# Matrixeigs/PowerSystemsReliabilityAssessment

Hardware: AMD Instinct MI355X
Metric: Monte Carlo DC-OPF scenarios/sec (RTS-24 HL2 non-sequential) (higher is better)
Workload: dtype f64

## Files before the change

### powersystemsreliabilityassessment_amd/_lib.py

```python
from __future__ import annotations

import ctypes as C
import os
import subprocess

from . import _abi

_CSRC = os.path.join(os.path.dirname(os.path.abspath(__file__)), "csrc")
LIB_PATH = os.environ.get("RELMC_LIB_PATH") or os.path.join(_CSRC, "librelmc.so")

EXPORTS = [
    "relmc_ctx_create", "relmc_ctx_destroy", "relmc_last_error", "relmc_version",
    "relmc_solver_opts_default", "relmc_nsq_opts_default", "relmc_case_load",
    "relmc_case_thresholds", "relmc_mc_sampling", "relmc_mc_sampling_dev",
    "relmc_mc_simulation", "relmc_mc_simulation_dev", "relmc_nsq_accumulate", "relmc_nsq_accumulate_distinct",
    "relmc_last_kernel_ms", "relmc_acc_zero", "relmc_acc_merge", "relmc_nsq_indices",
    "relmc_nsq_run", "relmc_hl1_load", "relmc_hl1_nsq", "relmc_hl1_seq_load", "relmc_hl1_seq", "relmc_hl1_seq_events",
    "relmc_hl1_plan_load", "relmc_hl1_plan", "relmc_hl1_area_load", "relmc_hl1_area", "relmc_hl1_area_tie_outages",
    "relmc_comm_unique_id", "relmc_comm_init", "relmc_comm_allreduce_acc", "relmc_comm_destroy", "relmc_comm_set_host_allreduce", "relmc_comm_info",
    "relmc_db_reset", "relmc_nsq_db_batch", "relmc_db_accumulate", "relmc_db_size", "relmc_db_export", "relmc_db_import",
    "relmc_seq_load", "relmc_seq_mcsampling", "relmc_seq_mcsimulation", "relmc_seq_years", "relmc_retry_stats", "relmc_retry_overflow", "relmc_retry_dense_stats", "relmc_case_order",
    "relmc_case_order_hint", "relmc_tune_order",
    "relmc_comm_set_timeout", "relmc_comm_allreduce_f64", "relmc_comm_set_host_allreduce_f64", "relmc_device_pci_bus_id", "relmc_seq_opts_default", "relmc_seq_run",
]
# ... 159 lines not shown
    L.relmc_tune_order.argtypes = [C.c_void_p, C.c_int32, C.c_uint64, i32p, i32p, i32p]
    L.relmc_tune_order.restype = C.c_int32
    L.relmc_db_export.argtypes = [vp, C.c_int64, C.c_int64, u8p, _abi.c_int64_p, dp, i32p, dp, i32p, i32p, u8p]
    L.relmc_db_export.restype = C.c_int32
    L.relmc_db_import.argtypes = [vp, C.c_void_p, C.c_int64, u8p, _abi.c_int64_p, dp, dp, i32p, i32p, u8p]
    L.relmc_db_import.restype = C.c_int32
    if hasattr(L, "relmc_debug_screen_states"):
        L.relmc_debug_screen_states.argtypes = [vp, u8p, dp, C.c_int64, u8p]
        L.relmc_debug_screen_states.restype = C.c_int32
    if hasattr(L, "relmc_debug_stretch_len"):
        L.relmc_debug_stretch_len.argtypes = [C.c_int64, C.c_int64, C.c_double, C.c_double, C.c_int64, i32p]
        L.relmc_debug_stretch_len.restype = C.c_int64
    if hasattr(L, "relmc_debug_set"):
        L.relmc_debug_set.argtypes = [vp, C.c_char_p, C.c_int32]
        L.relmc_debug_set.restype = C.c_int32
    if hasattr(L, "relmc_dpp_probe"):
        L.relmc_dpp_probe.argtypes = [vp, dp, dp]
        L.relmc_dpp_probe.restype = C.c_int32
    _lib = L
    return L
```

### powersystemsreliabilityassessment_amd/api.py

```python
from __future__ import annotations

import ctypes as C
from dataclasses import dataclass, field

import numpy as np

from . import _abi, _lib, case24

REFERENCE_EMULATE = _abi.RELMC_REFERENCE_EMULATE
PHYSICAL = _abi.RELMC_PHYSICAL


class RelmcError(RuntimeError):
    pass


def mpoption(singular_policy: int = REFERENCE_EMULATE, **overrides) -> _abi.SolverOpts:
    o = _abi.default_solver_opts(singular_policy)
    for k, v in overrides.items():
        if not hasattr(o, k):
            raise TypeError(f"unknown solver option {k!r}")
        setattr(o, k, v)
    return o

# ... 313 lines not shown
    def pci_bus_id(self) -> str:
        buf = C.create_string_buffer(64)
        self._check(self.L.relmc_device_pci_bus_id(self._h, buf, 64), "relmc_device_pci_bus_id")
        return buf.value.decode()

    def debug_set(self, key: str, value: bool = True):
        self._check(self.L.relmc_debug_set(self._h, key.encode(), int(bool(value))), "relmc_debug_set")

    def shape_path(self) -> str:
        f = self.L.relmc_debug_shape_path
        f.restype, f.argtypes = C.c_int32, [C.c_void_p]
        rc = f(self._h)
        if rc < 0:
            raise RelmcError(f"relmc_debug_shape_path failed ({rc})")
        return "static" if rc == 1 else "dynamic"

    def last_kernel_ms(self) -> float:
        ms = C.c_double()
        self._check(self.L.relmc_last_kernel_ms(self._h, C.byref(ms)), "relmc_last_kernel_ms")
        return ms.value

    def indices(self, acc: _abi.Acc, hours_per_year: float = 8760.0) -> _abi.Indices:
        out = _abi.Indices()
        self.L.relmc_nsq_indices(C.byref(acc), self.case.nb, self.case.ncomp, hours_per_year, C.byref(out))
        return out

    def nsqMain(self, beta_limit: float = 0.0017, max_iterations: int = 100000,
                samples_per_batch: int = 100, *, seed: int = 1, mpopt=None,
                hours_per_year: float = 8760.0, distinct_states: bool | int | str = False, verbose: bool = False) -> NsqResult:
        o = _abi.NsqOpts()
# ... 52 lines not shown
```

### powersystemsreliabilityassessment_amd/csrc/relmc_core.hip

```cpp
#include <hip/hip_runtime.h>

#include <cmath>
#include <cstddef>
#include <cstdio>
#include <cstdlib>
#include <cstring>
#include <memory>
#include <new>
#include <type_traits>

#include "relmc_ctx.h"
#ifdef RELMC_DEV_SWITCHES
#include "relmc_dev_switches.h"
#endif
#include "relmc_kernels.hip"

static_assert(sizeof(relmc::DevAcc) == sizeof(relmc_acc), "device accumulator image must match relmc_acc");

namespace relmc_host {

const char* const kNoCtx = "relmc: null context";

int fail(relmc_ctx* ctx, int code, const std::string& msg)
{
// ... 33 lines not shown
        HIP_TRY(ctx, ctx->retry.dense.grow(need));
        a.dense = ctx->retry.dense.get(); a.dense_stride = stride;
    }
    HIP_TRY(ctx, ctx->dpartial.grow(sizeof(PartialT<TL>) * 64 * TL::WPB * (size_t)blocks));
    a.partial = ctx->dpartial.get();
    a.scen_doubles = alt ? ctx->alt_scen_doubles[alt - 1] : ctx->scen_doubles;
    a.prio_mode = blocks != ctx->num_cu * ctx->blocks_per_cu ? 0u : (ctx->blocks_per_cu == 2 ? 1u : (ctx->blocks_per_cu == 1 && TL::WPB >= 8 ? 2u : 0u));
    a.stash_off = alt ? ctx->alt_stash_off[alt - 1] : ctx->stash_off;
    a.case_bytes = (uint32_t)offsetof(DevCaseT<TL>, task);
#if defined(RELMC_PHASE_TIMING) || defined(RELMC_TRACE)
    HIP_TRY(ctx, ctx->dtiming.grow(8 * 65536));
    a.timing = ctx->dtiming.get(); ctx->timing_waves = blocks * TL::WPB;
#else
    a.timing = nullptr;
#endif
    HIP_TRY(ctx, hipEventRecord(ev_start ? ev_start : ctx->ev0, ctx->stream));
    bool launched = false;
    if constexpr (MODE == 0 && std::is_same<TL, Tile24>::value) {
        if (alt == 0 && ctx->shape_static && !ctx->sw.dynamic_shape) {
            hipLaunchKernelGGL((relmc_eval_kernel<0, Tile24, ShapeRts24>), dim3(blocks), dim3(64 * Tile24::WPB), ctx->lds_bytes, ctx->stream,
                               reinterpret_cast<const DevCaseT<Tile24>*>(ctx->dcase.get()), a);
            launched = true;
        }
    }
    if (!launched)
        hipLaunchKernelGGL((relmc_eval_kernel<MODE, TL>), dim3(blocks), dim3(64 * TL::WPB), alt ? ctx->alt_lds_bytes[alt - 1] : ctx->lds_bytes, ctx->stream,
                           reinterpret_cast<const DevCaseT<TL>*>(alt ? ctx->dcase_alt[alt - 1].get() : ctx->dcase.get()), a);
    HIP_TRY(ctx, hipGetLastError());
    HIP_TRY(ctx, hipEventRecord(ev_stop ? ev_stop : ctx->ev1, ctx->stream));
    *rows_out = blocks * TL::WPB * TL::SPW;
    return RELMC_OK;
}

template <class TL>
int launch_eval_mode(relmc_ctx* ctx, int mode, EvalArgs& a, int* rows_out, hipEvent_t e0, hipEvent_t e1, int alt)
{
    switch (mode) {
        case 0: return launch_eval_t<0, TL>(ctx, a, rows_out, e0, e1, alt);
        case 1: return launch_eval_t<1, TL>(ctx, a, rows_out, e0, e1, alt);
        case 2: return launch_eval_t<2, TL>(ctx, a, rows_out, e0, e1, alt);
        case 3: return launch_eval_t<3, TL>(ctx, a, rows_out, e0, e1, alt);
        case 4: return launch_eval_t<4, TL>(ctx, a, rows_out, e0, e1, alt);
        case 5: return launch_eval_t<5, TL>(ctx, a, rows_out, e0, e1, alt);
// ... 102 lines not shown
    return case_load_impl<Tile96>(ctx, d, *C, order_variant);
}

namespace {
constexpr int64_t kProbeSamples = 8192;
int order_probe(relmc_ctx* ctx, int alt, int32_t* failures)
{
    relmc_solver_opts o; relmc_solver_opts_default(&o);
    EvalArgs a = make_args(o);
    a.seed = 0x5eedca5eull; a.first_index = 0; a.n = kProbeSamples;
    {
        const int rc0 = fail_list_ensure(ctx, fail_cap_for(kProbeSamples));
        if (rc0) return rc0;
    }
    auto& R = ctx->retry;
    HIP_TRY(ctx, hipMemsetAsync(R.fail_count.get(), 0, sizeof(uint32_t), ctx->stream));
    a.fail_list = R.fail.get(); a.fail_count = R.fail_count.get(); a.fail_cap = (uint32_t)R.fail.size(); a.unit_base = 0;
    int rows = 0;
    int rc = launch_eval(ctx, 5, a, &rows, nullptr, nullptr, alt);
    if (rc) return rc;
    uint32_t cnt = 0;
    HIP_TRY(ctx, hipMemcpyAsync(&cnt, R.fail_count.get(), sizeof(cnt), hipMemcpyDeviceToHost, ctx->stream));
    HIP_TRY(ctx, hipStreamSynchronize(ctx->stream));
    HIP_TRY(ctx, hipMemset(R.fail_count.get(), 0, sizeof(uint32_t)));
    R.fail_dirty = false;
    *failures = (int32_t)cnt;
    return RELMC_OK;
}

int order_calibrate(relmc_ctx* ctx)
{
    ctx->order_primary = 0; ctx->order_probe[0] = ctx->order_probe[1] = ctx->order_probe[2] = -1;
    if (ctx->sw.no_retry) return RELMC_OK;
    int rc = order_probe(ctx, 0, &ctx->order_probe[0]);
    if (rc) return rc;
    if ((int64_t)ctx->order_probe[0] * 1000 <= kProbeSamples) return RELMC_OK;
    int best = 0;
    for (int v = 0; v < relmc_ctx::kAlt; ++v) {
        if (alt_ensure(ctx, v) != RELMC_OK) continue;
// ... 257 lines not shown
```

### powersystemsreliabilityassessment_amd/csrc/relmc_ctx.h

```cpp
#pragma once
#include <hip/hip_runtime.h>

#include <cmath>
#include <cstdint>
#include <functional>
#include <string>
#include <vector>

#include "../../include/relmc.h"
#include "relmc_dev.h"

struct relmc_switches {
    bool no_retry = false;
    bool retry_dense_first = false;
    bool nsq_no_stretch = false;
    bool db_no_probe = false;
    bool dynamic_shape = false;
};

namespace relmc_host {
template <class T, bool Pinned = false>
class Buffer {
public:
    Buffer() = default;
    Buffer(Buffer&& o) noexcept : p_(o.p_), n_(o.n_) { o.p_ = nullptr; o.n_ = 0; }
    Buffer& operator=(Buffer&& o) noexcept
    {
        if (this != &o) { reset(); p_ = o.p_; n_ = o.n_; o.p_ = nullptr; o.n_ = 0; }
        return *this;
    }
    ~Buffer() { reset(); }
    T* get() const { return p_; }
// ... 29 lines not shown
    relmc_switches sw;
    struct SeqStep {
        DevBuf<uint32_t> dm, counts, off;
        DevBuf<uint16_t> hours; DevBuf<double> curt, year;
    } sq;
    std::vector<int32_t> order_hint;
    hipStream_t stream = nullptr;
    hipEvent_t ev0 = nullptr, ev1 = nullptr;
    bool has_case = false;
    int tile = 0;
    relmc::DevCaseT<relmc::Tile24> hcase24;
    relmc::DevCaseT<relmc::Tile96> hcase96;
    DevBuf<uint8_t> dcase;
    int nb = 0, ng = 0, nl = 0, ncomp = 0;
    DevBuf<uint8_t> dpartial;
    DevBuf<relmc::DevAcc> dacc;
    struct HostStage { relmc_acc acc; uint32_t fail_cnt, pad; };
    PinBuf<HostStage> hstage;
    int num_cu = 0;
    int blocks_per_cu = 0;
    uint32_t scen_doubles = 0, lds_bytes = 0, stash_off = 0;
    bool shape_static = false;
    DevBuf<unsigned long long> dtiming; int timing_waves = 0;
    struct History { DevBuf<double> d; PinBuf<double> h; } hist;
    struct Memo {
        DevBuf<uint32_t> k, perm0, perm1, head, uid, start, nu;
        DevBuf<unsigned long long> ch0, ch1; DevBuf<uint8_t> tmp;
        DevBuf<uint32_t> miss, k2;
    } memo;
    struct Database {
// ... 1 lines not shown
        DevBuf<uint32_t> keys; DevBuf<unsigned long long> count; DevBuf<double> dns; DevBuf<int32_t> meta; DevBuf<double> nodal; DevBuf<uint32_t> table;
        DevBuf<relmc::DevAcc> partial;
        DevBuf<unsigned long long> snap;
        bool has_opts = false; relmc_solver_opts opts = {};
        bool invalid = false;
    } db;
    struct CaseCopy {
        relmc_case_desc d; bool valid = false;
        std::vector<double> bus_pd, inj_pmin, inj_pmax, inj_cost, br_b, br_rate, unavail; std::vector<int32_t> inj_bus, br_from, br_to; std::vector<uint8_t> always_up;
    } case_copy;
    static constexpr int kAlt = 2;
    int alt_state[kAlt] = {0, 0};
    DevBuf<uint8_t> dcase_alt[kAlt]; uint32_t alt_scen_doubles[kAlt] = {0, 0}, alt_lds_bytes[kAlt] = {0, 0}, alt_stash_off[kAlt] = {0, 0};
    struct Retry {
        DevBuf<relmc::FailRec> fail; DevBuf<uint32_t> fail_count; bool fail_dirty = false;
        DevBuf<double> dense;
        DevBuf<uint32_t> keys; DevBuf<double> dns; DevBuf<int32_t> meta; DevBuf<double> nodal, scale; int64_t rows = 0;
    } retry;
    int64_t retry_dense_units = 0, retry_dense_converged = 0;
    int64_t retry_overflow = 0;
    std::vector<double> hlf;
    int64_t retry_units = 0, retry_converged = 0;
    int order_primary = 0; int32_t order_probe[3] = {-1, -1, -1};
    struct HostPipe {
        bool ready = false; int ncomp = 0, nb = 0;
        hipStream_t up = nullptr, down = nullptr;
        hipEvent_t e_up[2] = {nullptr, nullptr}, e_ks[2] = {nullptr, nullptr}, e_ke[2] = {nullptr, nullptr}, e_down[2] = {nullptr, nullptr};
        struct Bufs {
            DevBuf<uint8_t> d_st; DevBuf<double> d_sc, d_dns, d_nod; DevBuf<int32_t> d_stat, d_it;
            PinBuf<uint8_t> h_st; PinBuf<double> h_sc, h_dns, h_nod; PinBuf<int32_t> h_stat, h_it;
// ... 79 lines not shown
int case_symbolic(const relmc_case_desc* d, DevCaseT<TL>& C, int order_variant, const SymOpts& so, SymGeom& geom, std::string& err);
extern template int case_symbolic<Tile24>(const relmc_case_desc*, DevCaseT<Tile24>&, int, const SymOpts&, SymGeom&, std::string&);
extern template int case_symbolic<Tile96>(const relmc_case_desc*, DevCaseT<Tile96>&, int, const SymOpts&, SymGeom&, std::string&);
inline bool fits_tile24(const relmc_case_desc* d)
{
    return d->nb <= Tile24::NBT && d->nl <= Tile24::NLT && d->ng + d->nd <= Tile24::NIT && d->ng + d->nl <= Tile24::NCOMPMAX;
}

EvalArgs make_args(const relmc_solver_opts& o);
int launch_eval(relmc_ctx* ctx, int mode, EvalArgs& a, int* rows_out, hipEvent_t ev_start = nullptr, hipEvent_t ev_stop = nullptr, int alt = 0);
int launch_finalize(relmc_ctx* ctx, int rows);
int finish_timing(relmc_ctx* ctx);
int case_load_image(relmc_ctx* ctx, const relmc_case_desc* d, int order_variant);
inline int mask_words(const relmc_ctx* ctx) { return ctx->tile == 0 ? Tile24::OW : Tile96::OW; }

constexpr uint32_t kFailCapMin = 4096, kFailCapSteady = 1u << 20, kFailCapMax = 1u << 26;
uint32_t fail_cap_for(int64_t call_units);
int fail_list_ensure(relmc_ctx* ctx, uint32_t cap);
struct RetryOut { std::vector<FailRec> rec; std::vector<double> dns, nodal; std::vector<int32_t> meta; };
int alt_ensure(relmc_ctx* ctx, int v);
int fail_arm(relmc_ctx* ctx, EvalArgs& a, int64_t unit_base, bool reset, int64_t call_units);
int fail_listed(relmc_ctx* ctx, uint32_t* cnt);
using ScaleFn = std::function<double(unsigned long long)>;
int fail_retry(relmc_ctx* ctx, const relmc_solver_opts& o, double fail_threshold, const ScaleFn* scale, RetryOut& out, double* ms, const uint32_t* known_count = nullptr);
void acc_add_unit(relmc_acc* acc, const FailRec& rec, double dns, int32_t meta, const double* nodal, int nb, int ncomp, double fail_threshold);

int pipe_run(relmc_ctx* ctx, const uint8_t* states, const double* load_scale, int64_t n, const relmc_solver_opts& o, double fail_threshold,
             double* dns, double* nodal, int32_t* status, int32_t* iters);
int nsq_accumulate_impl(relmc_ctx* ctx, uint64_t seed, uint64_t first_index, int64_t n, const relmc_solver_opts* opts, relmc_acc* acc_out, double* dns_dev);

constexpr int64_t kStretch = 1 << 18, kStretchMaxBatch = 32768;
inline int64_t stretch_per(int64_t batch) { return kStretch / batch * batch; }
struct Stretch { int64_t len; bool final; };
// ... 38 lines not shown
```

### powersystemsreliabilityassessment_amd/csrc/relmc_debug.hip

```cpp
#include <cstdio>
#include <cstring>
#include <memory>

#include "relmc_ctx.h"
#include "relmc_shape_rts24.h"

using namespace relmc_host;

extern "C" {

int32_t relmc_debug_schedule(const relmc_ctx* ctx, int32_t* out9)
{
    if (!ctx || !out9 || !ctx->has_case) return RELMC_ERR_INVALID;
    auto fill = [&](const auto& C) {
        int ntask = 0;
        for (int p = 0; p < C.npass; ++p) ntask += C.pass_ntask[p];
        out9[0] = C.npass_upd; out9[1] = C.npass_inv; out9[2] = C.npass - C.npass_upd - C.npass_inv; out9[3] = C.noff;
        out9[4] = C.nzero; out9[5] = (int)C.nws; out9[6] = (int)ctx->lds_bytes; out9[7] = ctx->blocks_per_cu; out9[8] = ntask;
        if (verbose()) fprintf(stderr, "relmc: modelled LDS conflict cycles per Newton step %ld -> %ld\n", ctx->conflict_before, ctx->conflict_after);
        if (verbose()) fprintf(stderr, "relmc: longest line / injection list per bus slot: %d %d / %d %d\n", (int)C.maxdeg_s[0], (int)C.maxdeg_s[1], (int)C.maxinj_s[0], (int)C.maxinj_s[1]);
        if (verbose()) { fprintf(stderr, "relmc: tasks per pass:"); for (int p = 0; p < C.npass; ++p) fprintf(stderr, " %d", (int)C.pass_ntask[p]); fprintf(stderr, "\n"); }
    };
    if (ctx->tile == 0) fill(ctx->hcase24); else fill(ctx->hcase96);
    return RELMC_OK;
// ... 76 lines not shown

int64_t relmc_debug_stretch_len(int64_t batch, int64_t done, double beta, double beta_limit, int64_t round, int32_t* final_out)
{
    if (batch <= 0 || batch > kStretchMaxBatch || done < 0 || round < 0) return RELMC_ERR_INVALID;
    const Stretch s = stretch_length(batch, done, beta, beta_limit, stretch_per(batch), round);
    if (final_out) *final_out = s.final ? 1 : 0;
    return s.len;
}

int32_t relmc_debug_shape_path(const relmc_ctx* ctx)
{
    if (!ctx || !ctx->has_case) return RELMC_ERR_INVALID;
    return ctx->shape_static && !ctx->sw.dynamic_shape ? 1 : 0;
}

int32_t relmc_debug_set(relmc_ctx* ctx, const char* key, int32_t value)
{
    if (!ctx || !key) return RELMC_ERR_INVALID;
    const bool v = value != 0;
    if (!std::strcmp(key, "no_retry")) ctx->sw.no_retry = v;
    else if (!std::strcmp(key, "retry_dense_first")) ctx->sw.retry_dense_first = v;
    else if (!std::strcmp(key, "nsq_no_stretch")) ctx->sw.nsq_no_stretch = v;
    else if (!std::strcmp(key, "db_no_probe")) ctx->sw.db_no_probe = v;
    else if (!std::strcmp(key, "dynamic_shape")) ctx->sw.dynamic_shape = v;
    else return fail(ctx, RELMC_ERR_INVALID, std::string("relmc_debug_set: unknown switch ") + key);
    return RELMC_OK;
}

}
```

### powersystemsreliabilityassessment_amd/csrc/relmc_dev.h

```cpp
#pragma once
#include <stdint.h>

namespace relmc {

template <int RW_, int BS_, int LS_, int IS_, int NCOMPMAX_, int MAXPASS_, int MAXOFF_, int WPB_>
struct TileT {
    static constexpr int RW = RW_;
    static constexpr int BS = BS_;
    static constexpr int LS = LS_;
    static constexpr int IS = IS_;
    static constexpr int NBT = BS_ * RW_;
    static constexpr int NLT = LS_ * RW_;
    static constexpr int NIT = IS_ * RW_;
    static constexpr int SPW = 64 / RW_;
    static constexpr int NCOMPMAX = NCOMPMAX_;
    static constexpr int OW = NCOMPMAX_ / 32;
    static constexpr int MAXPASS = MAXPASS_;
    static constexpr int MAXOFF = MAXOFF_;
    static constexpr int WPB = WPB_;
    static_assert(BS_ <= 2 && LS_ <= 3 && IS_ <= 4, "the per-lane flag word has room for 2 bus, 3 line and 4 injection slots");
};
using Tile24 = TileT<16, 2, 3, 4, 128, 96, 160, 4>;
using Tile96 = TileT<64, 2, 2, 3, 256, 64, 320, 8>;
constexpr int DEGMAX = 8;
// ... 37 lines not shown
    uint16_t zero_off[MAXOFF];
    uint8_t pass_ntask[MAXPASS];
    uint16_t task[MAXPASS][ROWL][4];
};

template <class TL>
struct PartialT {
    double dns, dns2;
    double shed[TL::IS];
    uint32_t n, nfail, nsing, ninf, nnc, iters;
    uint32_t cf_inj[TL::IS];
    uint32_t cf_line[TL::LS];
    uint32_t pad;
};

struct FailRec {
    unsigned long long unit;
    uint32_t weight, pad;
    uint32_t mask[8];
};

struct EvalArgs {
    uint64_t seed, first_index;
    int64_t n;
    int32_t policy, max_it;
    double feastol, gradtol, comptol, costtol, xi, sigma, z0, alpha_min, max_stepsize;
    const uint8_t* states;
    double* dns;
    double* nodal;
    int32_t* status;
// ... 7 lines not shown
    double fail_threshold;
    const double* load_scale;
    const uint32_t* seq_masks;
    const uint32_t* seq_offsets;
    const uint16_t* seq_hours;
    const double* load_factors;
    double* curt;
    int32_t seq_nyears, seq_hpy;
    const uint32_t* memo_keys;
    const uint32_t* memo_perm;
    const uint32_t* memo_start;
    int64_t db_first;
    uint32_t* fail_count;
    FailRec* fail_list;
    uint32_t fail_cap;
    int64_t unit_base;
    double* dense;
    uint64_t dense_stride;
};

struct ScreenTab {
    int32_t nl, ng, valid, pad;
    double total_load;
    double sum_pmin, sum_rng;
    const double* pmin;
    const double* rng;
    const double* f_min;
    const double* f_rng;
    const double* f_load;
    const double* lim;
    const double* gpair;
    const double* hmat;
    const uint8_t* bridge;
// ... 75 lines not shown
```

### powersystemsreliabilityassessment_amd/csrc/relmc_kernels.hip

```cpp
#include "relmc_devfn.h"
#include "relmc_shape_rts24.h"

namespace relmc {


constexpr int kPrioBit = 12;
constexpr int kMinWaves = 2;
#define DINF __builtin_inf()
#define RELOAD_FENCE() __asm__ volatile("" ::: "memory")
#define SLOT_FENCE() __builtin_amdgcn_sched_barrier(0)
#ifdef RELMC_PASS_NOUNROLL
#define PASS_LOOP _Pragma("nounroll")
#else
#define PASS_LOOP
#endif
constexpr int kPfMask = 0xc0;
constexpr int kPfMaskWide = 0xc6;
#define PFSITE(k) (((PF_MASK >> (k)) & 1) != 0)
#ifdef RELMC_PHASE_TIMING
#define PT_DECL unsigned long long pt_[8] = {0, 0, 0, 0, 0, 0, 0, 0}; unsigned long long pt0_ = __builtin_readcyclecounter();
#define PT_MARK(k) { const unsigned long long n_ = __builtin_readcyclecounter(); pt_[k] += n_ - pt0_; pt0_ = n_; }
#define PT_FLUSH if (a.timing && lane == 0) { for (int k = 0; k < 8; ++k) a.timing[((size_t)blockIdx.x * WPB + (tid >> 6)) * 8 + k] = pt_[k]; }
#else
#define PT_DECL
// ... 91 lines not shown
    PT_DECL
    const int64_t ngroups = (a.n + SPW - 1) / SPW;
    const int64_t gwave = (int64_t)blockIdx.x * WPB + (tid >> 6);
    const int64_t gstride = (int64_t)gridDim.x * WPB;
    const bool prio_first = a.prio_mode == 1 ? blockIdx.x < (gridDim.x >> 1) : (a.prio_mode == 2 ? ((tid >> 8) & 1) == 0 : false);
    if (a.prio_mode != 0 && !prio_first) __builtin_amdgcn_s_setprio(1);
    constexpr bool WINDOWED = (MODE == 0 && RW == 16);
    uint32_t* const WIN = reinterpret_cast<uint32_t*>(smem + OPT_BYTES + ((case_bytes + 15u) & ~15u)) +
                          (size_t)SPW * WPB * SHAPE(scen_doubles, a.scen_doubles) * 2 + (size_t)(tid >> 6) * 256;
    uint8_t* const WINL = reinterpret_cast<uint8_t*>(smem + OPT_BYTES + ((case_bytes + 15u) & ~15u)) +
                          ((size_t)SPW * WPB * SHAPE(scen_doubles, a.scen_doubles) * 2 + (size_t)WPB * 256) * 4 + (size_t)(tid >> 6) * 64;
    int64_t wb_begin = gwave, wb_end = ngroups, wb_step = gstride;
    if (WINDOWED) {
        wb_begin = ngroups * gwave / gstride; wb_end = ngroups * (gwave + 1) / gstride; wb_step = 16;
    }
    for (int64_t wb = wb_begin; wb < wb_end; wb += wb_step) {
    int win_groups = 1;
    uint32_t win_valid = 0;
    if (WINDOWED) {
        const int64_t si = wb * 4 + lane;
        const bool valid = (wb + (lane >> 2)) < wb_end && si < a.n;
        uint32_t m0 = 0, m1 = 0, m2 = 0, m3 = 0;
        bool hard = false;
        if (valid) {
            const uint64_t gi = a.first_index + (uint64_t)si;
            const int nblk = (ncomp + 3) >> 2;
            for (int blk = 0; blk < nblk; ++blk) {
                uint32_t w[4], nib = 0;
                philox4x32_10((uint32_t)gi, (uint32_t)(gi >> 32), (uint32_t)blk, 0u, (uint32_t)a.seed, (uint32_t)(a.seed >> 32), w);
#pragma unroll
                for (int e = 0; e < 4; ++e) {
                    const int k = blk * 4 + e;
                    if (k < ncomp && w[e] < C.thr[k]) nib |= 1u << e;
                }
// ... 8 lines not shown
            }
            hard = cap * base < C.total_load;
        }
        const uint64_t bv = __ballot(valid), bh = __ballot(valid && hard);
        const uint64_t below = (1ull << lane) - 1ull;
        const uint32_t n_valid = (uint32_t)__popcll(bv), n_easy = (uint32_t)__popcll(bv & ~bh);
        if (valid) {
            const uint32_t slot = hard ? n_easy + (uint32_t)__popcll(bh & below) : (uint32_t)__popcll(bv & ~bh & below);
            uint4 pk; pk.x = m0; pk.y = m1; pk.z = m2; pk.w = m3;
            *reinterpret_cast<uint4*>(WIN + 4 * slot) = pk;
            WINL[slot] = (uint8_t)lane;
        }
        RELOAD_FENCE();
        win_valid = n_valid;
        win_groups = (int)((n_valid + 3u) >> 2);
    }
    PT_IMARK(0)
    for (int wg = 0; wg < win_groups; ++wg) {
        const int64_t grp = WINDOWED ? wb + wg : wb;
        const int64_t sidx = grp * SPW + lane / RW;
        const bool live = WINDOWED ? (uint32_t)(wg * 4 + lane / RW) < win_valid : sidx < a.n;
        double lscale = 1.0;
        uint32_t wgt = 1;
        int seq_year = 0, seq_hour = 0;
        RELOAD_FENCE();

        uint32_t sf = 0;
#define L_ON(s) (((sf >> (s)) & 1u) != 0)
#define L_ACT(s) (((sf >> (3 + (s))) & 1u) != 0)
#define I_ON(s) (((sf >> (6 + (s))) & 1u) != 0)
#define I_BOX(s) (((sf >> (10 + (s))) & 1u) != 0)
#define B_PIN(t) (((sf >> (14 + (t))) & 1u) != 0)
#define B_DROP(t) (((sf >> (16 + (t))) & 1u) != 0)
// ... 883 lines not shown
                    }
#pragma unroll
                    for (int t = 0; t < BS; ++t) {
                        bth[t] = __builtin_fma(alphap, dth[t], bth[t]); bla[t] = __builtin_fma(alphad, dla[t], bla[t]);
                        if (vb[t] < nb) Lam[vb[t]] = bla[t];
                    }
                    zmu = row_sum<RW>(zl);
                    fval = row_sum<RW>(fl);
                    if (niq > 0) gamma = (PFSITE(6) ? o_sg : A_(5, sigma)) * zmu / (double)niq;
                }
                PT_MARK(6)
            }
        }

        PT_MARK(6)
        if (live) {
            double dns = fval + C.total_load * lscale;
            if (dns < 0.1) dns = 0.0;
            const bool fail = dns > a.fail_threshold;
            bool defer = false;
            if (a.fail_list && (status == 1 || status == 2)) {
                uint32_t pos = 0;
                if (rlane == 0) pos = atomicAdd(a.fail_count, 1u);
                pos = __shfl(pos, lane & ~(RW - 1));
                if (pos < a.fail_cap) {
                    defer = true;
                    FailRec* fr = a.fail_list + pos;
                    if (rlane < OW) fr->mask[rlane] = OB[rlane];
                    if (rlane == 0) {
                        const int64_t u = (MODE == 0 && WINDOWED) ? wb * 4 + WINL[wg * 4 + lane / RW]
// ... 1 lines not shown
                                          : (MODE == 7 ? (int64_t)a.memo_perm[sidx]
                                          : (MODE == 4 && a.memo_perm ? (int64_t)a.memo_perm[sidx] : sidx)));
                        fr->unit = (unsigned long long)(u + a.unit_base); fr->weight = wgt; fr->pad = 0;
                    }
                }
            }
            double shed[IS];
#pragma unroll
            for (int s = 0; s < IS; ++s) {
                const int j = RW * s + rlane;
                shed[s] = 0.0;
                if (((iinfo[s] >> 8) & 0xff) == IK_VIRTUAL && dns > 0.0) {
                    const double v = ip[s] * base - C.i_tab[j][3] * lscale;
                    if (v > 1e-3) shed[s] = v;
                }
                if (MODE != 4 && !defer && shed[s] != 0.0) PA.shed[s] += MODE == 3 ? shed[s] * (double)wgt : shed[s];
                if (MODE != 4 && !defer && fail && ((iinfo[s] >> 8) & 0xff) == IK_REAL && outbit(OB, j)) PA.cf_inj[s] += wgt;
            }
#pragma unroll
            for (int s = 0; s < LS; ++s)
                if (MODE != 4 && !defer && fail && ((linfo[s] >> 24) & LF_EXISTS) && outbit(OB, ng + RW * s + rlane)) PA.cf_line[s] += wgt;
            if (MODE != 4 && !defer && rlane == 0) {
                acc_n += wgt;
                if (dns != 0.0) {
                    if (MODE == 3) { PA.dns = __builtin_fma((double)wgt, dns, PA.dns); PA.dns2 = __builtin_fma((double)wgt * dns, dns, PA.dns2); }
                    else { PA.dns += dns; PA.dns2 = __builtin_fma(dns, dns, PA.dns2); }
                }
                if (fail) PA.nfail += wgt;
                if (status == 3) PA.nsing += wgt;
                if (status == 1 || status == 2) PA.nnc += wgt;
                if (infeas) PA.ninf += wgt;
                acc_it += (uint32_t)it * wgt;
            }
            if (MODE == 2 && rlane == 0) a.curt[(size_t)seq_year * a.seq_hpy + seq_hour] = dns;
            if (MODE == 0 && a.dns && rlane == 0)
                a.dns[WINDOWED ? wb * 4 + WINL[wg * 4 + lane / RW] : sidx] = dns;
            if (MODE == 7 && a.dns && rlane == 0) a.dns[a.memo_perm[sidx]] = dns;
            if (MODE == 1 || MODE == 4) {
                const int64_t oidx = MODE == 4 ? a.db_first + (a.memo_perm ? (int64_t)a.memo_perm[sidx] : sidx) : sidx;
#pragma unroll
                for (int s = 0; s < IS; ++s) if (RW * s + rlane < nip) IR[4 * (RW * s + rlane)] = shed[s];
                if (rlane == 0) {
                    a.dns[oidx] = dns;
                    if (MODE == 4) a.status[oidx] = status | (infeas ? 4 : 0) | (it << 8);
                    else {
                        if (a.status) a.status[oidx] = status;
                        if (a.iters) a.iters[oidx] = it;
                    }
                }
                if (a.nodal) {
#pragma unroll
                    for (int t = 0; t < BS; ++t) {
                        const int i = vb[t];
                        if (i < nb) {
                            const int vj = C.b_vinj[i];
                            a.nodal[oidx * nb + C.b_ext[i]] = vj >= 0 ? IR[4 * vj] : 0.0;
                        }
                    }
                }
            }
        }
        PT_MARK(7)
    }
    }
    if (rlane == 0) { PA.n = acc_n; PA.iters = acc_it; }
    PT_FLUSH
}

constexpr int FIN_THREADS = 256, FIN_UNROLL = 8;
template <class TL>
__global__ void __launch_bounds__(FIN_THREADS) relmc_finalize_kernel(const DevCaseT<TL>* __restrict__ C, const PartialT<TL>* __restrict__ part,
                                                                     int nrows, DevAcc* __restrict__ out)
{
    constexpr int RW = TL::RW;
    using Partial = PartialT<TL>;
    const int item = blockIdx.x, tid = threadIdx.x;
    int ln = 0; size_t foff = 0;
    bool is_int = true, active = true;
    if (item < 6) foff = offsetof(Partial, n) + sizeof(uint32_t) * (size_t)item;
    else if (item < 8) { foff = item == 6 ? offsetof(Partial, dns) : offsetof(Partial, dns2); is_int = false; }
    else if (item < 8 + 256) {
// ... 92 lines not shown
```

### powersystemsreliabilityassessment_amd/csrc/relmc_retry.hip

```cpp
#include <algorithm>
#include <cstring>

#include "relmc_ctx.h"

namespace relmc_host {

uint32_t fail_cap_for(int64_t call_units)
{
    const int64_t c = (int64_t)kFailCapMin + call_units / 256;
    return c > (int64_t)kFailCapSteady ? kFailCapSteady : (uint32_t)c;
}
int fail_list_ensure(relmc_ctx* ctx, uint32_t cap)
{
    auto& R = ctx->retry;
    if (!R.fail_count.get()) {
        HIP_TRY(ctx, R.fail_count.grow(1));
        HIP_TRY(ctx, hipMemsetAsync(R.fail_count.get(), 0, sizeof(uint32_t), ctx->stream));
    }
    if (cap <= R.fail.size()) return RELMC_OK;
    HIP_TRY(ctx, hipStreamSynchronize(ctx->stream));
    HIP_TRY(ctx, R.fail.grow(cap));
    return RELMC_OK;
}

int alt_ensure(relmc_ctx* ctx, int v)
{
    if (ctx->alt_state[v]) return ctx->alt_state[v] > 0 ? RELMC_OK : RELMC_ERR_UNSUPPORTED;
    ctx->alt_state[v] = -1;
    if (!ctx->case_copy.valid) return RELMC_ERR_UNSUPPORTED;
    const std::string keep = ctx->err;
    const int rc = case_load_image(ctx, &ctx->case_copy.d, v + 1);
    ctx->err = keep;
    if (rc == RELMC_OK) ctx->alt_state[v] = 1;
    return rc;
}

int fail_arm(relmc_ctx* ctx, EvalArgs& a, int64_t unit_base, bool reset, int64_t call_units)
{
    a.fail_list = nullptr; a.fail_count = nullptr; a.fail_cap = 0; a.unit_base = unit_base;
    if (ctx->sw.no_retry) return RELMC_OK;
    if (reset || !ctx->retry.fail.get()) {
        const int rc = fail_list_ensure(ctx, fail_cap_for(call_units));
        if (rc) return rc;
    }
    if (reset && ctx->retry.fail_dirty) { HIP_TRY(ctx, hipMemsetAsync(ctx->retry.fail_count.get(), 0, sizeof(uint32_t), ctx->stream)); }
    if (reset) ctx->retry.fail_dirty = true;
    a.fail_list = ctx->retry.fail.get(); a.fail_count = ctx->retry.fail_count.get(); a.fail_cap = (uint32_t)ctx->retry.fail.size();
    return RELMC_OK;
}

int fail_listed(relmc_ctx* ctx, uint32_t* cnt)
{
    *cnt = 0;
    if (!ctx->retry.fail_count.get()) return RELMC_OK;
    HIP_TRY(ctx, hipMemcpy(cnt, ctx->retry.fail_count.get(), sizeof(*cnt), hipMemcpyDeviceToHost));
    return RELMC_OK;
}

int fail_retry(relmc_ctx* ctx, const relmc_solver_opts& o, double fail_threshold, const ScaleFn* scale_fn, RetryOut& out, double* ms, const uint32_t* known_count)
{
    const bool have_scale = scale_fn != nullptr;
    auto scale = [&](unsigned long long u) { return (*scale_fn)(u); };
    out.rec.clear();
    if (!ctx->retry.fail_count.get()) return RELMC_OK;
    uint32_t cnt = 0;
    if (known_count) cnt = *known_count;
    else HIP_TRY(ctx, hipMemcpy(&cnt, ctx->retry.fail_count.get(), sizeof(cnt), hipMemcpyDeviceToHost));
    ctx->retry.fail_dirty = false;
    if (cnt == 0) return RELMC_OK;
    HIP_TRY(ctx, hipMemset(ctx->retry.fail_count.get(), 0, sizeof(uint32_t)));
    const uint32_t cap = (uint32_t)ctx->retry.fail.size();
    if (cnt > cap) {
        ctx->retry_overflow += (int64_t)(cnt - cap);
        cnt = cap;
    }
    out.rec.resize(cnt);
    HIP_TRY(ctx, hipMemcpy(out.rec.data(), ctx->retry.fail.get(), sizeof(FailRec) * cnt, hipMemcpyDeviceToHost));
    std::sort(out.rec.begin(), out.rec.end(), [](const FailRec& x, const FailRec& y) { return x.unit < y.unit; });
    const int ow = ctx->tile == 0 ? Tile24::OW : Tile96::OW;
    const size_t nb = (size_t)ctx->nb;
    auto& R = ctx->retry;
    if ((int64_t)cnt > R.rows) { R.rows = kFailCapMin; while (R.rows < (int64_t)cnt) R.rows *= 2; }
    const size_t rc2 = (size_t)R.rows;
    HIP_TRY(ctx, R.keys.grow(rc2 * 2 * 8));
    HIP_TRY(ctx, R.dns.grow(rc2 * 2));
// ... 122 lines not shown
```

### powersystemsreliabilityassessment_amd/csrc/relmc_simulate.hip

```cpp
#include <cmath>
#include <cstring>
#include <thread>

#include "relmc_ctx.h"

namespace relmc_host {

constexpr int64_t kPipeChunk = 131072;

int pipe_ensure(relmc_ctx* ctx)
{
    auto& P = ctx->pipe;
    if (P.ready && P.ncomp == ctx->ncomp && P.nb == ctx->nb) return RELMC_OK;
    P.ready = false;
    if (!P.up) HIP_TRY(ctx, hipStreamCreateWithFlags(&P.up, hipStreamNonBlocking));
    if (!P.down) HIP_TRY(ctx, hipStreamCreateWithFlags(&P.down, hipStreamNonBlocking));
    for (int b = 0; b < 2; ++b)
        for (hipEvent_t* e : {&P.e_up[b], &P.e_ks[b], &P.e_ke[b], &P.e_down[b]}) if (!*e) HIP_TRY(ctx, hipEventCreate(e));
    const size_t c = (size_t)kPipeChunk, nc = (size_t)ctx->ncomp, nb = (size_t)ctx->nb;
    bool ok = true;
    for (auto& B : P.buf) {
        B = {};
        ok = ok && B.d_st.grow(c * nc) == hipSuccess && B.d_sc.grow(c) == hipSuccess && B.d_dns.grow(c) == hipSuccess && B.d_nod.grow(c * nb) == hipSuccess &&
             B.d_stat.grow(c) == hipSuccess && B.d_it.grow(c) == hipSuccess && B.h_st.grow(c * nc) == hipSuccess && B.h_sc.grow(c) == hipSuccess &&
// ... 117 lines not shown
        for (int attempt = 0; a.n > 0; ++attempt) {
            int rc = fail_arm(ctx, a, done, true, m);
            if (rc) return rc;
            rc = launch_eval(ctx, screen ? 7 : 0, a, &blocks);
            if (rc) return rc;
            rc = launch_finalize(ctx, blocks);
            if (rc) return rc;
            HIP_TRY(ctx, hipMemcpyAsync(&ctx->hstage.get()->acc, ctx->dacc.get(), sizeof(relmc_acc), hipMemcpyDeviceToHost, ctx->stream));
            if (a.fail_count) HIP_TRY(ctx, hipMemcpyAsync(&ctx->hstage.get()->fail_cnt, ctx->retry.fail_count.get(), sizeof(uint32_t), hipMemcpyDeviceToHost, ctx->stream));
            rc = finish_timing(ctx);
            if (rc) return rc;
            ms_total += ctx->last_kernel_ms;
            part = ctx->hstage.get()->acc;
            listed = a.fail_count ? ctx->hstage.get()->fail_cnt : 0u;
            if (a.fail_list == nullptr || listed <= ctx->retry.fail.size() || ctx->retry.fail.size() >= kFailCapMax || attempt >= 2) break;
            HIP_TRY(ctx, hipMemset(ctx->retry.fail_count.get(), 0, sizeof(uint32_t)));
            rc = fail_list_ensure(ctx, listed + listed / 8 > kFailCapMax ? kFailCapMax : listed + listed / 8);
            if (rc) return rc;
        }
        part.n += certified; part.n_screened += certified;
        int rc = RELMC_OK;
        RetryOut ro;
        if (a.n > 0) rc = fail_retry(ctx, o, a.fail_threshold, nullptr, ro, &ms_total, a.fail_count ? &listed : nullptr);
        if (rc) return rc;
        for (size_t r = 0; r < ro.rec.size(); ++r) {
            acc_add_unit(&part, ro.rec[r], ro.dns[r], ro.meta[r], &ro.nodal[r * (size_t)ctx->nb], ctx->nb, ctx->ncomp, a.fail_threshold);
            if (dns_dev) HIP_TRY(ctx, hipMemcpy(dns_dev + ro.rec[r].unit, &ro.dns[r], sizeof(double), hipMemcpyHostToDevice));
        }
        relmc_acc_merge(acc_out, &part);
        done += m;
    }
// ... 66 lines not shown
```

Baseline: 59.31 million.

## Add dynamic tail work-stealing with parked partials replayed by a follow-up kernel

```diff
diff --git a/powersystemsreliabilityassessment_amd/_lib.py b/powersystemsreliabilityassessment_amd/_lib.py
--- a/powersystemsreliabilityassessment_amd/_lib.py
+++ b/powersystemsreliabilityassessment_amd/_lib.py
@@ -197,6 +197,11 @@
     if hasattr(L, "relmc_debug_set"):
         L.relmc_debug_set.argtypes = [vp, C.c_char_p, C.c_int32]
         L.relmc_debug_set.restype = C.c_int32
+    if hasattr(L, "relmc_debug_tail_plan"):
+        L.relmc_debug_tail_plan.argtypes = [C.c_int64, C.c_int32, C.c_void_p, C.c_void_p, C.c_void_p, C.c_void_p]
+        L.relmc_debug_tail_plan.restype = C.c_int32
+        L.relmc_debug_tail_groups.argtypes = [vp, _abi.c_int64_p, i32p]
+        L.relmc_debug_tail_groups.restype = C.c_int32
     if hasattr(L, "relmc_dpp_probe"):
         L.relmc_dpp_probe.argtypes = [vp, dp, dp]
         L.relmc_dpp_probe.restype = C.c_int32
diff --git a/powersystemsreliabilityassessment_amd/api.py b/powersystemsreliabilityassessment_amd/api.py
--- a/powersystemsreliabilityassessment_amd/api.py
+++ b/powersystemsreliabilityassessment_amd/api.py
@@ -351,6 +351,13 @@
         if rc < 0:
             raise RelmcError(f"relmc_debug_shape_path failed ({rc})")
         return "static" if rc == 1 else "dynamic"
+
+    def tail_groups(self):
+        k, w = C.c_int64(), C.c_int32()
+        t = self.L.relmc_debug_tail_groups(self._h, C.byref(k), C.byref(w))
+        if t < 0:
+            raise RelmcError(f"relmc_debug_tail_groups failed ({t})")
+        return int(t), int(k.value), int(w.value)
 
     def last_kernel_ms(self) -> float:
         ms = C.c_double()
diff --git a/powersystemsreliabilityassessment_amd/csrc/relmc_core.hip b/powersystemsreliabilityassessment_amd/csrc/relmc_core.hip
--- a/powersystemsreliabilityassessment_amd/csrc/relmc_core.hip
+++ b/powersystemsreliabilityassessment_amd/csrc/relmc_core.hip
@@ -71,6 +71,19 @@
 #else
     a.timing = nullptr;
 #endif
+    a.tail_groups = 0;
+    if constexpr (MODE == 0 && std::is_same<TL, Tile24>::value) {
+        a.tail_rec = nullptr; a.tail_count = nullptr;
+        const TailPlan plan(a.n, (int64_t)blocks * TL::WPB);
+        if (plan.T > 0 && !ctx->sw.static_tail) {
+            { const int rc = fail_count_ensure(ctx); if (rc) return rc; }
+            HIP_TRY(ctx, ctx->dtail.grow(sizeof(TailRecT<TL>) * (size_t)plan.items()));
+            a.tail_groups = plan.T; a.tail_rec = ctx->dtail.get(); a.tail_count = ctx->retry.fail_count.get() + 1;
+        }
+        ctx->last_tail_groups = a.tail_groups; ctx->tail_launches += a.tail_groups > 0;
+        if (verbose()) fprintf(stderr, "relmc: fused launch of %lld scenarios on %d wavefronts: tail groups T = %d%s\n", (long long)a.n, blocks * TL::WPB, a.tail_groups,
+                               a.tail_groups ? "" : (ctx->sw.static_tail ? " (static_tail)" : " (fewer than 2 T groups per wavefront)"));
+    }
     HIP_TRY(ctx, hipEventRecord(ev_start ? ev_start : ctx->ev0, ctx->stream));
     bool launched = false;
     if constexpr (MODE == 0 && std::is_same<TL, Tile24>::value) {
@@ -84,6 +97,13 @@
         hipLaunchKernelGGL((relmc_eval_kernel<MODE, TL>), dim3(blocks), dim3(64 * TL::WPB), alt ? ctx->alt_lds_bytes[alt - 1] : ctx->lds_bytes, ctx->stream,
                            reinterpret_cast<const DevCaseT<TL>*>(alt ? ctx->dcase_alt[alt - 1].get() : ctx->dcase.get()), a);
     HIP_TRY(ctx, hipGetLastError());
+    if constexpr (MODE == 0 && std::is_same<TL, Tile24>::value) {
+        if (a.tail_groups > 0) {
+            hipLaunchKernelGGL(relmc_tail_replay_kernel<TL>, dim3(blocks), dim3(64 * TL::WPB), 0, ctx->stream, reinterpret_cast<PartialT<TL>*>(ctx->dpartial.get()),
+                               reinterpret_cast<const TailRecT<TL>*>(ctx->dtail.get()), a.tail_groups, a.tail_count);
+            HIP_TRY(ctx, hipGetLastError());
+        }
+    }
     HIP_TRY(ctx, hipEventRecord(ev_stop ? ev_stop : ctx->ev1, ctx->stream));
     *rows_out = blocks * TL::WPB * TL::SPW;
     return RELMC_OK;
@@ -216,7 +236,7 @@
         if (rc0) return rc0;
     }
     auto& R = ctx->retry;
-    HIP_TRY(ctx, hipMemsetAsync(R.fail_count.get(), 0, sizeof(uint32_t), ctx->stream));
+    HIP_TRY(ctx, hipMemsetAsync(R.fail_count.get(), 0, R.kCountBytes, ctx->stream));
     a.fail_list = R.fail.get(); a.fail_count = R.fail_count.get(); a.fail_cap = (uint32_t)R.fail.size(); a.unit_base = 0;
     int rows = 0;
     int rc = launch_eval(ctx, 5, a, &rows, nullptr, nullptr, alt);
@@ -224,7 +244,7 @@
     uint32_t cnt = 0;
     HIP_TRY(ctx, hipMemcpyAsync(&cnt, R.fail_count.get(), sizeof(cnt), hipMemcpyDeviceToHost, ctx->stream));
     HIP_TRY(ctx, hipStreamSynchronize(ctx->stream));
-    HIP_TRY(ctx, hipMemset(R.fail_count.get(), 0, sizeof(uint32_t)));
+    HIP_TRY(ctx, hipMemset(R.fail_count.get(), 0, R.kCountBytes));
     R.fail_dirty = false;
     *failures = (int32_t)cnt;
     return RELMC_OK;
diff --git a/powersystemsreliabilityassessment_amd/csrc/relmc_ctx.h b/powersystemsreliabilityassessment_amd/csrc/relmc_ctx.h
--- a/powersystemsreliabilityassessment_amd/csrc/relmc_ctx.h
+++ b/powersystemsreliabilityassessment_amd/csrc/relmc_ctx.h
@@ -16,6 +16,7 @@
     bool nsq_no_stretch = false;
     bool db_no_probe = false;
     bool dynamic_shape = false;
+    bool static_tail = false;
 };
 
 namespace relmc_host {
@@ -75,6 +76,8 @@
     DevBuf<uint8_t> dcase;
     int nb = 0, ng = 0, nl = 0, ncomp = 0;
     DevBuf<uint8_t> dpartial;
+    DevBuf<uint8_t> dtail;
+    int last_tail_groups = 0; int64_t tail_launches = 0;
     DevBuf<relmc::DevAcc> dacc;
     struct HostStage { relmc_acc acc; uint32_t fail_cnt, pad; };
     PinBuf<HostStage> hstage;
@@ -106,6 +109,7 @@
     DevBuf<uint8_t> dcase_alt[kAlt]; uint32_t alt_scen_doubles[kAlt] = {0, 0}, alt_lds_bytes[kAlt] = {0, 0}, alt_stash_off[kAlt] = {0, 0};
     struct Retry {
         DevBuf<relmc::FailRec> fail; DevBuf<uint32_t> fail_count; bool fail_dirty = false;
+        static constexpr size_t kCountWords = 2, kCountBytes = kCountWords * sizeof(uint32_t);
         DevBuf<double> dense;
         DevBuf<uint32_t> keys; DevBuf<double> dns; DevBuf<int32_t> meta; DevBuf<double> nodal, scale; int64_t rows = 0;
     } retry;
@@ -215,9 +219,25 @@
 int case_load_image(relmc_ctx* ctx, const relmc_case_desc* d, int order_variant);
 inline int mask_words(const relmc_ctx* ctx) { return ctx->tile == 0 ? Tile24::OW : Tile96::OW; }
 
+#ifndef RELMC_TAIL_GROUPS
+#define RELMC_TAIL_GROUPS 8
+#endif
+constexpr int kTailGroups = RELMC_TAIL_GROUPS;
+struct TailPlan {
+    int64_t ngroups, waves; int T;
+    TailPlan(int64_t n, int64_t waves_) : ngroups((n + Tile24::SPW - 1) / Tile24::SPW), waves(waves_), T(waves_ > 0 && ngroups / waves_ >= 2 * kTailGroups ? kTailGroups : 0) {}
+    int64_t begin(int64_t w) const { return ngroups * w / waves; }
+    int64_t end(int64_t w) const { return ngroups * (w + 1) / waves; }
+    int64_t cut(int64_t w) const { return end(w) - T; }
+    int64_t items() const { return waves * T; }
+    int64_t owner(int64_t p) const { return p % waves; }
+    int64_t group(int64_t p) const { return end(p % waves) - T + p / waves; }
+};
+
 constexpr uint32_t kFailCapMin = 4096, kFailCapSteady = 1u << 20, kFailCapMax = 1u << 26;
 uint32_t fail_cap_for(int64_t call_units);
 int fail_list_ensure(relmc_ctx* ctx, uint32_t cap);
+int fail_count_ensure(relmc_ctx* ctx);
 struct RetryOut { std::vector<FailRec> rec; std::vector<double> dns, nodal; std::vector<int32_t> meta; };
 int alt_ensure(relmc_ctx* ctx, int v);
 int fail_arm(relmc_ctx* ctx, EvalArgs& a, int64_t unit_base, bool reset, int64_t call_units);
diff --git a/powersystemsreliabilityassessment_amd/csrc/relmc_debug.hip b/powersystemsreliabilityassessment_amd/csrc/relmc_debug.hip
--- a/powersystemsreliabilityassessment_amd/csrc/relmc_debug.hip
+++ b/powersystemsreliabilityassessment_amd/csrc/relmc_debug.hip
@@ -114,6 +114,23 @@
     return ctx->shape_static && !ctx->sw.dynamic_shape ? 1 : 0;
 }
 
+int32_t relmc_debug_tail_plan(int64_t n, int32_t waves, int64_t* a_begin, int64_t* a_end, int32_t* owner, int64_t* group)
+{
+    if (n < 0 || waves <= 0) return RELMC_ERR_INVALID;
+    const TailPlan plan(n, waves);
+    for (int64_t w = 0; w < waves; ++w) { if (a_begin) a_begin[w] = plan.begin(w); if (a_end) a_end[w] = plan.cut(w); }
+    for (int64_t p = 0; p < plan.items(); ++p) { if (owner) owner[p] = (int32_t)plan.owner(p); if (group) group[p] = plan.group(p); }
+    return plan.T;
+}
+
+int32_t relmc_debug_tail_groups(const relmc_ctx* ctx, int64_t* launches_out, int32_t* waves_out)
+{
+    if (!ctx) return RELMC_ERR_INVALID;
+    if (launches_out) *launches_out = ctx->tail_launches;
+    if (waves_out) *waves_out = ctx->has_case && ctx->tile == 0 ? ctx->num_cu * ctx->blocks_per_cu * Tile24::WPB : 0;
+    return ctx->last_tail_groups;
+}
+
 int32_t relmc_debug_set(relmc_ctx* ctx, const char* key, int32_t value)
 {
     if (!ctx || !key) return RELMC_ERR_INVALID;
@@ -123,6 +140,7 @@
     else if (!std::strcmp(key, "nsq_no_stretch")) ctx->sw.nsq_no_stretch = v;
     else if (!std::strcmp(key, "db_no_probe")) ctx->sw.db_no_probe = v;
     else if (!std::strcmp(key, "dynamic_shape")) ctx->sw.dynamic_shape = v;
+    else if (!std::strcmp(key, "static_tail")) ctx->sw.static_tail = v;
     else return fail(ctx, RELMC_ERR_INVALID, std::string("relmc_debug_set: unknown switch ") + key);
     return RELMC_OK;
 }
diff --git a/powersystemsreliabilityassessment_amd/csrc/relmc_dev.h b/powersystemsreliabilityassessment_amd/csrc/relmc_dev.h
--- a/powersystemsreliabilityassessment_amd/csrc/relmc_dev.h
+++ b/powersystemsreliabilityassessment_amd/csrc/relmc_dev.h
@@ -75,6 +75,13 @@
     uint32_t pad;
 };
 
+template <class TL>
+struct TailRecT {
+    double shed[64][TL::IS];
+    double dns[TL::SPW];
+    uint32_t flag[TL::SPW];
+};
+
 struct FailRec {
     unsigned long long unit;
     uint32_t weight, pad;
@@ -112,9 +119,10 @@
     uint32_t* fail_count;
     FailRec* fail_list;
     uint32_t fail_cap;
+    int32_t tail_groups;
     int64_t unit_base;
-    double* dense;
-    uint64_t dense_stride;
+    union { double* dense; void* tail_rec; };
+    union { uint64_t dense_stride; uint32_t* tail_count; };
 };
 
 struct ScreenTab {
diff --git a/powersystemsreliabilityassessment_amd/csrc/relmc_kernels.hip b/powersystemsreliabilityassessment_amd/csrc/relmc_kernels.hip
--- a/powersystemsreliabilityassessment_amd/csrc/relmc_kernels.hip
+++ b/powersystemsreliabilityassessment_amd/csrc/relmc_kernels.hip
@@ -129,10 +129,34 @@
     if (WINDOWED) {
         wb_begin = ngroups * gwave / gstride; wb_end = ngroups * (gwave + 1) / gstride; wb_step = 16;
     }
-    for (int64_t wb = wb_begin; wb < wb_end; wb += wb_step) {
-    int win_groups = 1;
+    static_assert(!WINDOWED || 80 + 4 * WPB <= OPT_BYTES, "one word per wavefront behind the ten option doubles");
+    int* const TP = reinterpret_cast<int*>(smem + 80) + (tid >> 6);
+    if (WINDOWED) { *TP = -1; RELOAD_FENCE(); }
+    for (int64_t wb = wb_begin; WINDOWED || wb < wb_end; wb += wb_step) {
+    int win_groups = 1, wg0 = 0;
     uint32_t win_valid = 0;
     if (WINDOWED) {
+        const int T = a.tail_groups;
+        int run = 16;
+        if (__builtin_amdgcn_readfirstlane((int)(*TP < 0 && wb < wb_end - T)) != 0) {
+            if (wb_end - T - wb < 16) run = (int)(wb_end - T - wb);
+        } else {
+            if (T == 0) break;
+            uint32_t p = 0;
+            if (lane == 0) p = atomicAdd(a.tail_count, 1u);
+            p = __builtin_amdgcn_readfirstlane(p);
+            int64_t n_ = a.n; uint32_t nw = gridDim.x;
+            __asm__ volatile("" : "+s"(n_), "+s"(nw));
+            nw *= WPB;
+            if (p >= nw * (uint32_t)T) break;
+            const int64_t ng_ = (n_ + SPW - 1) / SPW, owner = p % nw, ob = ng_ * owner / nw;
+            wb_end = ng_ * (owner + 1) / nw;
+            const int64_t g = wb_end - T + p / nw;
+            wb = ob + ((g - ob) & ~(int64_t)15);
+            wg0 = (int)(g - wb); run = wg0 + 1;
+            *TP = (int)p;
+            RELOAD_FENCE();
+        }
         const int64_t si = wb * 4 + lane;
         const bool valid = (wb + (lane >> 2)) < wb_end && si < a.n;
         uint32_t m0 = 0, m1 = 0, m2 = 0, m3 = 0;
@@ -171,9 +195,10 @@
         RELOAD_FENCE();
         win_valid = n_valid;
         win_groups = (int)((n_valid + 3u) >> 2);
+        if (run < win_groups) win_groups = run;
     }
     PT_IMARK(0)
-    for (int wg = 0; wg < win_groups; ++wg) {
+    for (int wg = wg0; wg < win_groups; ++wg) {
         const int64_t grp = WINDOWED ? wb + wg : wb;
         const int64_t sidx = grp * SPW + lane / RW;
         const bool live = WINDOWED ? (uint32_t)(wg * 4 + lane / RW) < win_valid : sidx < a.n;
@@ -1087,6 +1112,11 @@
         }
 
         PT_MARK(6)
+        using TailRec = TailRecT<TL>;
+        RELOAD_FENCE();
+        const int tp = WINDOWED ? *TP : -1;
+        const bool park = WINDOWED && tp >= 0;
+        uint32_t tflag = 0;
         if (live) {
             double dns = fval + C.total_load * lscale;
             if (dns < 0.1) dns = 0.0;
@@ -1118,7 +1148,7 @@
                     const double v = ip[s] * base - C.i_tab[j][3] * lscale;
                     if (v > 1e-3) shed[s] = v;
                 }
-                if (MODE != 4 && !defer && shed[s] != 0.0) PA.shed[s] += MODE == 3 ? shed[s] * (double)wgt : shed[s];
+                if (MODE != 4 && !defer && !park && shed[s] != 0.0) PA.shed[s] += MODE == 3 ? shed[s] * (double)wgt : shed[s];
                 if (MODE != 4 && !defer && fail && ((iinfo[s] >> 8) & 0xff) == IK_REAL && outbit(OB, j)) PA.cf_inj[s] += wgt;
             }
 #pragma unroll
@@ -1128,6 +1158,7 @@
                 acc_n += wgt;
                 if (dns != 0.0) {
                     if (MODE == 3) { PA.dns = __builtin_fma((double)wgt, dns, PA.dns); PA.dns2 = __builtin_fma((double)wgt * dns, dns, PA.dns2); }
+                    else if (park) { reinterpret_cast<TailRec*>(a.tail_rec)[tp].dns[lane / RW] = dns; tflag = 1; }
                     else { PA.dns += dns; PA.dns2 = __builtin_fma(dns, dns, PA.dns2); }
                 }
                 if (fail) PA.nfail += wgt;
@@ -1135,6 +1166,11 @@
                 if (status == 1 || status == 2) PA.nnc += wgt;
                 if (infeas) PA.ninf += wgt;
                 acc_it += (uint32_t)it * wgt;
+            }
+            if (WINDOWED && park && !defer && dns != 0.0) {
+                double* const ts = reinterpret_cast<TailRec*>(a.tail_rec)[tp].shed[lane];
+#pragma unroll
+                for (int s = 0; s < IS; ++s) ts[s] = shed[s];
             }
             if (MODE == 2 && rlane == 0) a.curt[(size_t)seq_year * a.seq_hpy + seq_hour] = dns;
             if (MODE == 0 && a.dns && rlane == 0)
@@ -1164,11 +1200,33 @@
                 }
             }
         }
+        if (WINDOWED && park && rlane == 0) reinterpret_cast<TailRec*>(a.tail_rec)[tp].flag[lane / RW] = tflag;
         PT_MARK(7)
     }
     }
     if (rlane == 0) { PA.n = acc_n; PA.iters = acc_it; }
     PT_FLUSH
+}
+
+template <class TL>
+__global__ void __launch_bounds__(64 * TL::WPB) relmc_tail_replay_kernel(PartialT<TL>* __restrict__ part, const TailRecT<TL>* __restrict__ rec, int tail_groups,
+                                                                           uint32_t* __restrict__ tail_count)
+{
+    constexpr int RW = TL::RW, IS = TL::IS, WPB = TL::WPB;
+    const int tid = threadIdx.x, lane = tid & 63;
+    const size_t nw = (size_t)gridDim.x * WPB, owner = (size_t)blockIdx.x * WPB + (tid >> 6);
+    PartialT<TL>& PA = part[(size_t)blockIdx.x * (64 * WPB) + tid];
+    for (int k = 0; k < tail_groups; ++k) {
+        const TailRecT<TL>& R = rec[(size_t)k * nw + owner];
+        if (R.flag[lane / RW] == 0) continue;
+#pragma unroll
+        for (int s = 0; s < IS; ++s) { const double v = R.shed[lane][s]; if (v != 0.0) PA.shed[s] += v; }
+        if ((lane & (RW - 1)) == 0) {
+            const double dns = R.dns[lane / RW];
+            if (dns != 0.0) { PA.dns += dns; PA.dns2 = __builtin_fma(dns, dns, PA.dns2); }
+        }
+    }
+    if (blockIdx.x == 0 && tid == 0) *tail_count = 0u;
 }
 
 constexpr int FIN_THREADS = 256, FIN_UNROLL = 8;
diff --git a/powersystemsreliabilityassessment_amd/csrc/relmc_retry.hip b/powersystemsreliabilityassessment_amd/csrc/relmc_retry.hip
--- a/powersystemsreliabilityassessment_amd/csrc/relmc_retry.hip
+++ b/powersystemsreliabilityassessment_amd/csrc/relmc_retry.hip
@@ -10,13 +10,19 @@
     const int64_t c = (int64_t)kFailCapMin + call_units / 256;
     return c > (int64_t)kFailCapSteady ? kFailCapSteady : (uint32_t)c;
 }
-int fail_list_ensure(relmc_ctx* ctx, uint32_t cap)
+int fail_count_ensure(relmc_ctx* ctx)
 {
     auto& R = ctx->retry;
     if (!R.fail_count.get()) {
-        HIP_TRY(ctx, R.fail_count.grow(1));
-        HIP_TRY(ctx, hipMemsetAsync(R.fail_count.get(), 0, sizeof(uint32_t), ctx->stream));
-    }
+        HIP_TRY(ctx, R.fail_count.grow(R.kCountWords));
+        HIP_TRY(ctx, hipMemsetAsync(R.fail_count.get(), 0, R.kCountBytes, ctx->stream));
+    }
+    return RELMC_OK;
+}
+int fail_list_ensure(relmc_ctx* ctx, uint32_t cap)
+{
+    auto& R = ctx->retry;
+    { const int rc = fail_count_ensure(ctx); if (rc) return rc; }
     if (cap <= R.fail.size()) return RELMC_OK;
     HIP_TRY(ctx, hipStreamSynchronize(ctx->stream));
     HIP_TRY(ctx, R.fail.grow(cap));
@@ -43,7 +49,7 @@
         const int rc = fail_list_ensure(ctx, fail_cap_for(call_units));
         if (rc) return rc;
     }
-    if (reset && ctx->retry.fail_dirty) { HIP_TRY(ctx, hipMemsetAsync(ctx->retry.fail_count.get(), 0, sizeof(uint32_t), ctx->stream)); }
+    if (reset && ctx->retry.fail_dirty) { HIP_TRY(ctx, hipMemsetAsync(ctx->retry.fail_count.get(), 0, ctx->retry.kCountBytes, ctx->stream)); }
     if (reset) ctx->retry.fail_dirty = true;
     a.fail_list = ctx->retry.fail.get(); a.fail_count = ctx->retry.fail_count.get(); a.fail_cap = (uint32_t)ctx->retry.fail.size();
     return RELMC_OK;
@@ -68,7 +74,7 @@
     else HIP_TRY(ctx, hipMemcpy(&cnt, ctx->retry.fail_count.get(), sizeof(cnt), hipMemcpyDeviceToHost));
     ctx->retry.fail_dirty = false;
     if (cnt == 0) return RELMC_OK;
-    HIP_TRY(ctx, hipMemset(ctx->retry.fail_count.get(), 0, sizeof(uint32_t)));
+    HIP_TRY(ctx, hipMemset(ctx->retry.fail_count.get(), 0, ctx->retry.kCountBytes));
     const uint32_t cap = (uint32_t)ctx->retry.fail.size();
     if (cnt > cap) {
         ctx->retry_overflow += (int64_t)(cnt - cap);
diff --git a/powersystemsreliabilityassessment_amd/csrc/relmc_simulate.hip b/powersystemsreliabilityassessment_amd/csrc/relmc_simulate.hip
--- a/powersystemsreliabilityassessment_amd/csrc/relmc_simulate.hip
+++ b/powersystemsreliabilityassessment_amd/csrc/relmc_simulate.hip
@@ -155,7 +155,7 @@
             part = ctx->hstage.get()->acc;
             listed = a.fail_count ? ctx->hstage.get()->fail_cnt : 0u;
             if (a.fail_list == nullptr || listed <= ctx->retry.fail.size() || ctx->retry.fail.size() >= kFailCapMax || attempt >= 2) break;
-            HIP_TRY(ctx, hipMemset(ctx->retry.fail_count.get(), 0, sizeof(uint32_t)));
+            HIP_TRY(ctx, hipMemset(ctx->retry.fail_count.get(), 0, ctx->retry.kCountBytes));
             rc = fail_list_ensure(ctx, listed + listed / 8 > kFailCapMax ? kFailCapMax : listed + listed / 8);
             if (rc) return rc;
         }
```

Result: faster. 61.24 million, median of 6 (+3.2%).
